# url-kaist/UV-SLAM

Hardware: AMD Instinct MI355X
Metric: sliding-window solves/sec (10 KF, 150 pts, 40 lines, 3 VP) (higher is better)
Workload: dtype f64; 1 GPU; W10-P150-L40-V3 x 256 independent windows per GPU (BASELINE configs[2]); single window (configs[1]) in single_window, the 20k-point window (configs[3]) in large_window (both with --full); windows_per_gpu=256, frames=11, points=150, lines=40, vp_tagged_lines=30, prior=True, parallelism=replicas x1

## Files before the change

### uv-slam_amd/csrc/uvs_solve_kernel.h

```cpp
#pragma once
#include <hip/hip_runtime.h>
#include "../../include/uvs_solver.h"
#include "uvs_layout.h"
#include "uvs_factors.h"

namespace uvsdev {


#ifndef UVS_X_PLAIN_TID
static __device__ __forceinline__ int lane_tid() { int t = threadIdx.x; asm volatile("" : "+v"(t)); return t; }
#else
static __device__ __forceinline__ int lane_tid() { return threadIdx.x; }
#endif
static constexpr int NT = UVS_NT;
static constexpr int NW = NT / 64;
static constexpr bool ROLES = NT > 256;
static constexpr int ET = ROLES ? 256 : NT;
static constexpr int EW = ET / 64;
static constexpr int GT0 = NT - UVS_GT;
UVS_DEV int wave_uniform() { return __builtin_amdgcn_readfirstlane((int)(threadIdx.x >> 6)); }
UVS_DEV bool role_eval() { return !ROLES || wave_uniform() < EW; }
#ifndef UVS_X_NO_LINE_ROTATE
UVS_DEV int line_lane() { return ROLES ? (lane_tid() ^ 256) : lane_tid(); }
#else
UVS_DEV int line_lane() { return lane_tid(); }
#endif
#define UVS_COST_LINE_LANE tid
#ifndef UVS_T_CP_PB
#define UVS_T_CP_PB 2
#define UVS_T_CP_LB 1
#define UVS_T_BS_LNB 4
#define UVS_T_PR_UN 26
#endif
static_assert(UVS_PT_C == UVS_PT_A + 12, "pt_anchor_pass reads A and c as one run");
static constexpr int CP_PB = NT > 256 ? UVS_T_CP_PB : 4;
static constexpr int CP_LB = NT > 256 ? UVS_T_CP_LB : 2;
static constexpr int BS_LNB = NT > 256 ? UVS_T_BS_LNB : 4;
static constexpr int PR_UN = NT > 256 ? UVS_T_PR_UN : 26;
static constexpr int PG_UN = NT > 256 ? 16 : 32;

static constexpr int L_X = 0;
static constexpr int L_XC = L_X + UVS_XDIM;
static constexpr int L_G = L_XC + UVS_XDIM;
static constexpr int L_DLT = L_G + UVS_RD;
static constexpr int L_HD = L_DLT + UVS_RD + 24;
static constexpr int L_SC = L_HD + UVS_RD;
static constexpr int L_DD = L_SC + UVS_RD;
static constexpr int L_DINV = L_DD + UVS_RD;
static constexpr int L_RF = L_DINV + UVS_RD;
static constexpr int L_EX = L_RF + 120;
static constexpr int L_PDX = L_EX + 16;
static constexpr int L_PR = L_PDX + UVS_MAX_PRIOR_DIM;
static constexpr int L_PRC = L_PR + UVS_MAX_PRIOR_DIM;
static constexpr int L_RED = L_PRC + UVS_MAX_PRIOR_DIM;
static constexpr int L_CTRL = L_RED + (5 * NW > 24 ? 5 * NW : 24);
static constexpr int L_PROF = L_CTRL + 32;
static constexpr int L_WPROF = L_PROF + 24;
static constexpr int L_LCOST = L_WPROF + 8;
static constexpr int LACC = 1;
static constexpr int L_LGMAX = L_LCOST + ET / LACC;
static constexpr int L_PX0 = L_LGMAX + 8;
static constexpr int L_PTAB = L_PX0 + 9 * UVS_MAX_PRIOR_BLOCKS;
static constexpr int L_SMALL = (L_PTAB + 2 * UVS_MAX_PRIOR_BLOCKS + 1) & ~1;
static constexpr int L_S = L_SMALL;
static constexpr int L_TOTAL = L_S + UVS_S_DOUBLES;
static_assert(L_TOTAL * 8 <= 160 * 1024, "LDS map exceeds the 160 KB of a CU");
enum { P_SETUP = 0, P_OBS, P_LMPREP, P_GATHER, P_ASSEMBLE, P_CHOL, P_TRSV, P_BACKSUB, P_COST, P_MISC, P_CH_DIAG, P_CH_PANEL, P_CH_TRAIL, P_AS_IMU, P_AS_ZERO, P_AS_ADD, P_LAST };
#define UVS_PROF(c, k) do { if ((c).o.debug && lane_tid() == 0) { const long long now_ = clock64(); (c).sh[L_PROF + (k)] += (double)(now_ - (long long)(c).sh[L_PROF + 23]); (c).sh[L_PROF + 23] = (double)now_; } } while (0)
static constexpr size_t LDS_BYTES = (size_t)L_TOTAL * 8;
static constexpr int TL_PER_WAVE = 4096;
__device__ long long g_lin_tl[8 * TL_PER_WAVE * 2];
#define UVS_TLOG(c, id) do { if ((c).o.debug == 5 && (threadIdx.x & 63) == 0 && blockIdx.x == 0) { const int w_ = threadIdx.x >> 6; const int n_ = (int)(c).sh[L_WPROF + w_]; \
    if (n_ < TL_PER_WAVE) { g_lin_tl[2 * (w_ * TL_PER_WAVE + n_)] = (id); g_lin_tl[2 * (w_ * TL_PER_WAVE + n_) + 1] = clock64(); (c).sh[L_WPROF + w_] = (double)(n_ + 1); } } } while (0)

enum { C_COST = 0, C_RADIUS, C_DECR, C_XNORM, C_GMAX, C_CAND, C_MCC, C_STEP2, C_XC2, C_GO, C_IT, C_INVALID, C_CUR, C_FIRST,
       C_TERM, C_NSUCC, C_CHOLOK, C_GMAXLM, C_TIMEUP };

struct KOpts {
    int max_it, ex_free, keep_cand, jacobi;
    double sqrt_info, line_factor, vp_factor, loss_pt, loss_ln, loss_vp, G[3];
    double r0, rmax, rmin, min_rel, dlo, dhi, ftol, gtol, ptol;
    int max_invalid;
    int debug;
    long long max_ticks;
    int redamp;
};

__constant__ unsigned char c_blk_fa[UVS_NBLK];
__constant__ unsigned char c_blk_fb[UVS_NBLK];

UVS_DEV int sidx(int i, int j) {
    const int bi = i >> 4, bj = j >> 4;
    return (((bi * (bi + 1)) >> 1) + bj) * UVS_BLK_SZ + (i & 15) * UVS_BLK_LD + (j & 15);
}
UVS_DEV double bcast_lane(double v, int lane) {
    const int lo = __builtin_amdgcn_readlane(__double2loint(v), lane);
    const int hi = __builtin_amdgcn_readlane(__double2hiint(v), lane);
    return __hiloint2double(hi, lo);
}
UVS_DEV void wave_sync() {
    __builtin_amdgcn_fence(__ATOMIC_RELEASE, "wavefront");
    __builtin_amdgcn_wave_barrier();
    __builtin_amdgcn_fence(__ATOMIC_ACQUIRE, "wavefront");
}

UVS_DEV double wave_sum(double v) {
#pragma unroll
    for (int off = 32; off > 0; off >>= 1) v += __shfl_down(v, off, 64);
    return v;
}
UVS_DEV double wave_max(double v) {
#pragma unroll
    for (int off = 32; off > 0; off >>= 1) v = fmax(v, __shfl_down(v, off, 64));
    return v;
}
UVS_DEV void rsqrt_pair(double x, double* sq, double* rsq) {
    const double y = __builtin_amdgcn_rsq(x);
    double g = x * y, hh = 0.5 * y;
    double r = fma(-hh, g, 0.5);
    g = fma(g, r, g); hh = fma(hh, r, hh);
    r = fma(-hh, g, 0.5);
    g = fma(g, r, g); hh = fma(hh, r, hh);
    const double d = fma(-g, g, x);
    g = fma(d, hh, g);
    *sq = g; *rsq = 2.0 * hh;
}
UVS_DEV void block_reduce(double* sh, double* s , double* mx) {
    const int tid = lane_tid(), lane = tid & 63, wv = tid >> 6;
    __syncthreads();
#pragma unroll
    for (int k = 0; k < 4; ++k) { const double t = wave_sum(s[k]); if (lane == 0) sh[L_RED + wv * 5 + k] = t; }
    { const double t = wave_max(*mx); if (lane == 0) sh[L_RED + wv * 5 + 4] = t; }
    __syncthreads();
    double a[4] = {0, 0, 0, 0}, m = 0.0;
#pragma unroll
    for (int w = 0; w < NW; ++w) {
#pragma unroll
        for (int k = 0; k < 4; ++k) a[k] += sh[L_RED + w * 5 + k];
        m = fmax(m, sh[L_RED + w * 5 + 4]);
    }
#pragma unroll
    for (int k = 0; k < 4; ++k) s[k] = a[k];
    *mx = m;
}

UVS_DEV void lacc_set(double* sh, double cost, double gmax) {
    const int tid = lane_tid();
    if (tid < ET) sh[L_LCOST + tid] = cost;
    const double wm = wave_max(gmax);
    if ((tid & 63) == 0) sh[L_LGMAX + (tid >> 6)] = wm;
}
UVS_DEV void lacc_add(double* sh, double cost, double gmax) {
    const int tid = lane_tid();
    if (tid < ET) sh[L_LCOST + tid] += cost;
    const double wm = wave_max(gmax);
    if ((tid & 63) == 0) sh[L_LGMAX + (tid >> 6)] = fmax(sh[L_LGMAX + (tid >> 6)], wm);
}
UVS_DEV double lacc_cost(const double* sh) { const int tid = lane_tid(); return tid < ET ? sh[L_LCOST + tid] : 0.0; }
UVS_DEV double lacc_gmax(const double* sh) { return sh[L_LGMAX + (lane_tid() >> 6)]; }

struct Ctx {
    const DevWin* hdr;
    const double* bd;
    const int* bi;
    double* ws;
    double* sh;
    KOpts o;
    int ltrig_ok = 0;
    int ptab_ok = 0;
};

UVS_DEV const double* line_trig_of(const Ctx& c, const double* line) {
    const DevWin& h = *c.hdr;
    if (!c.ltrig_ok) return nullptr;
    return line == c.ws + h.w_line0 ? c.ws + h.w_ltrig0 : (line == c.ws + h.w_line1 ? c.ws + h.w_ltrig1 : nullptr);
}

UVS_DEV void stage_rotations(const Ctx& c, const double* x) {
    const int tid = lane_tid();
    if (tid < UVS_NF) quat_to_R(x + 7 * tid + 3, c.sh + L_RF + 9 * tid);
    else if (tid == UVS_NF) { quat_to_R(x + 176 + 3, c.sh + L_EX); c.sh[L_EX + 9] = x[176]; c.sh[L_EX + 10] = x[177]; c.sh[L_EX + 11] = x[178]; }
    else if (tid == UVS_RELO_FRAME && c.hdr->relo_on) quat_to_R(x + 184 + 3, c.sh + L_RF + 9 * UVS_RELO_FRAME);
}
UVS_DEV const double* pose_of(const double* x, int f) { return x + (f > UVS_NF ? 184 : 7 * f); }

UVS_DEV void load_point_obs(const Ctx& c, int o, double td, double* pi, double* pj, double* vij) {
    const DevWin& h = *c.hdr;
    const double* m = c.bd + h.d_ptmeas + o; const int st = h.pt_stride;
    pi[0] = m[0]; pi[1] = m[st]; pi[2] = m[2 * st]; pj[0] = m[3 * st]; pj[1] = m[4 * st]; pj[2] = m[5 * st];
    if (h.td_on) {
        const double* v = c.bd + h.d_ptvel + o;
        vij[0] = v[0]; vij[1] = v[st]; vij[2] = v[2 * st]; vij[3] = v[3 * st];
        const double di = td - v[4 * st], dj = td - v[5 * st];
        pi[0] -= di * vij[0]; pi[1] -= di * vij[1]; pj[0] -= dj * vij[2]; pj[1] -= dj * vij[3];
    }
}

UVS_DEV void stage_prior_tables(const Ctx& c) {
    const int tid = lane_tid();
    const DevWin& h = *c.hdr;
    if (h.prior_n <= 0) return;
    int* tab = (int*)(c.sh + L_PTAB);
    if (tid < 4 * UVS_MAX_PRIOR_BLOCKS) tab[tid] = c.bi[h.i_prior + tid];
    if (tid < 9 * UVS_MAX_PRIOR_BLOCKS) c.sh[L_PX0 + tid] = c.bd[h.d_prior + h.prior_n * h.prior_n + 2 * h.prior_n + tid];
}
UVS_DEV void prior_dx(const Ctx& c, const double* x) {
    const int tid = lane_tid() - 64;
    const DevWin& h = *c.hdr;
    if (h.prior_n > 0 && tid >= 0 && tid < h.prior_nb) {
        int kind, frame, size, idx;
        double x0[9];
        if (c.ptab_ok) {
            const int* tab = (const int*)(c.sh + L_PTAB);
            kind = tab[tid]; frame = tab[16 + tid]; size = tab[32 + tid]; idx = tab[48 + tid];
#pragma unroll
            for (int k = 0; k < 9; ++k) x0[k] = c.sh[L_PX0 + 9 * tid + k];
        } else {
            const int* pt = c.bi + h.i_prior;
            kind = pt[tid]; frame = pt[16 + tid]; size = pt[32 + tid]; idx = pt[48 + tid];
            const double* x0g = c.bd + h.d_prior + h.prior_n * h.prior_n + 2 * h.prior_n + 9 * tid;
#pragma unroll
            for (int k = 0; k < 9; ++k) x0[k] = x0g[k];
        }
        const double* xb = (kind == UVS_BLOCK_POSE) ? x + 7 * frame : (kind == UVS_BLOCK_SPEEDBIAS) ? x + 77 + 9 * frame : (kind == UVS_BLOCK_TD) ? x + 183 : x + 176;
        double* dx = c.sh + L_PDX + idx;
        if (size != 7) { for (int k = 0; k < size; ++k) dx[k] = xb[k] - x0[k]; }
        else {
            dx[0] = xb[0] - x0[0]; dx[1] = xb[1] - x0[1]; dx[2] = xb[2] - x0[2];
            double qi[4], e[4]; quat_inv(x0 + 3, qi); quat_mul(qi, xb + 3, e);
            const double sg = (e[3] >= 0.0) ? 2.0 : -2.0;
            dx[3] = sg * e[0]; dx[4] = sg * e[1]; dx[5] = sg * e[2];
        }
    }
}
UVS_DEV double prior_quad(const Ctx& c, int dst = L_PR) {
    const DevWin& h = *c.hdr;
    const int n = h.prior_n, tid = lane_tid();
    double cost = 0.0;
    if (n <= 0) return cost;
    const double* H0 = c.ws + h.w_prior_h0;
    const int parts = (NT / n) < 4 ? (NT / n) : 4;
    const int part = tid / n, row = tid - part * n;
    const double g0v = tid < n ? c.ws[h.w_prior_h0 + UVS_PH_G0(n) + tid] : 0.0, c0v = tid == 0 ? c.ws[h.w_prior_h0 + UVS_PH_C0(n)] : 0.0;
    if (part < parts) {
        const int kb = (n * part) / parts, ke = (n * (part + 1)) / parts;
        double p8[8] = {0, 0, 0, 0, 0, 0, 0, 0};
        for (int k = kb; k < ke; k += PR_UN) {
            double jv[PR_UN];
#pragma unroll
            for (int u = 0; u < PR_UN; ++u) jv[u] = H0[(k + u < ke ? k + u : kb) * n + row];
#pragma unroll
            for (int u = 0; u < PR_UN; ++u) if (k + u < ke) p8[u & 7] += jv[u] * c.sh[L_PDX + k + u];
        }
        c.sh[L_S + 128 * part + row] = ((p8[0] + p8[1]) + (p8[2] + p8[3])) + ((p8[4] + p8[5]) + (p8[6] + p8[7]));
    }
    __syncthreads();
    if (tid < n) {
        double y = c.sh[L_S + tid];
        for (int p = 1; p < parts; ++p) y += c.sh[L_S + 128 * p + tid];
        c.sh[dst + tid] = y;
        cost = c.sh[L_PDX + tid] * (g0v + 0.5 * y);
        if (tid == 0) cost += c0v;
    }
    return cost;
}
UVS_DEV double prior_cost_share(const Ctx& c, int src) {
    const DevWin& h = *c.hdr;
    const int n = h.prior_n, tid = lane_tid();
    double cost = 0.0;
    if (tid < n) {
        cost = c.sh[L_PDX + tid] * (c.ws[h.w_prior_h0 + UVS_PH_G0(n) + tid] + 0.5 * c.sh[src + tid]);
        if (tid == 0) cost += c.ws[h.w_prior_h0 + UVS_PH_C0(n)];
    }
    return cost;
}
UVS_DEV double prior_residual_rows(const Ctx& c) {
    const DevWin& h = *c.hdr;
    const int n = h.prior_n, tid = lane_tid();
    double cost = 0.0;
    if (tid < n) {
        const double* Jr = c.bd + h.d_prior + (size_t)tid * n;
        double s = c.bd[h.d_prior + n * n + tid];
        for (int k = 0; k < n; ++k) s += Jr[k] * c.sh[L_PDX + k];
        c.sh[L_PR + tid] = s;
        cost = 0.5 * s * s;
    }
    return cost;
}

UVS_DEV void cost_imu_raw(const Ctx& c, const double* x, int lane0) {
    const DevWin& h = *c.hdr;
    const int b = lane_tid() - lane0;
    double* rs = c.sh + L_S + 1024;
    if (b >= 0 && b < h.n_imu) {
        const int fi = c.bi[h.i_imu + 2 * b], skip = c.bi[h.i_imu + 2 * b + 1];
        if (!skip) {
            const double* blk = c.bd + h.d_imu + (size_t)b * UVS_IMU_STRIDE;
            double r[15];
            imu_raw(blk, blk + UVS_IMU_JAC, c.o.G, x + 7 * fi, x + 77 + 9 * fi, x + 7 * (fi + 1), x + 77 + 9 * (fi + 1), r, nullptr);
#pragma unroll
            for (int i = 0; i < 15; ++i) rs[16 * b + i] = r[i];
        }
    }
}
// ... 213 lines not shown
    double a0[4], b0[4], a1[4], b1[4];
#define UVS_CH_LOAD(AV, BV) { _Pragma("unroll") for (int q = 0; q < 4; ++q) { AV[q] = Ai[4 * q]; BV[q] = Bj[4 * q]; } Bj += UVS_BLK_SZ; Ai += astep; }
#define UVS_CH_MFMA(AV, BV) { _Pragma("unroll") for (int q = 0; q < 4; ++q) acc = TR ? __builtin_amdgcn_mfma_f64_16x16x4f64(BV[q], AV[q], acc, 0, 0, 1) : __builtin_amdgcn_mfma_f64_16x16x4f64(AV[q], BV[q], acc, 0, 0, 1); }
    UVS_CH_LOAD(a0, b0)
    for (int j = j0;;) {
        if (j + 1 < j1) UVS_CH_LOAD(a1, b1)
        UVS_CH_MFMA(a0, b0)
        if (++j >= j1) break;
        if (j + 1 < j1) UVS_CH_LOAD(a0, b0)
        UVS_CH_MFMA(a1, b1)
        if (++j >= j1) break;
    }
#undef UVS_CH_LOAD
#undef UVS_CH_MFMA
}
template <bool RHS>
UVS_DEV void chol_panel_pair(double* sh, int i1, int i2, int k, int lane, const double* Bw, const d4_t& av) {
    d4_t acc = {0.0, 0.0, 0.0, 0.0};
#pragma unroll
    for (int q = 0; q < 4; ++q) acc = __builtin_amdgcn_mfma_f64_16x16x4f64(av[q], Bw[q], acc, 0, 0, 0);
    chol_store_pair<RHS>(sh, i1, i2, k, lane, acc);
}

UVS_DEV void chol_panel_item(double* sh, int i, int k, int lane, const double* Bw) {
    const int li = lane & 15, lk = lane >> 4;
    d4_t acc = {0.0, 0.0, 0.0, 0.0};
    double av[4];
    if (i != UVS_NF) {
        const double* Ai = sblk(sh, i, k) + li * UVS_BLK_LD + lk;
#pragma unroll
        for (int q = 0; q < 4; ++q) av[q] = Ai[4 * q];
    } else {
#pragma unroll
        for (int q = 0; q < 4; ++q) { const double yv = sh[L_DLT + 16 * k + 4 * q + lk]; av[q] = (li == 0) ? yv : 0.0; }
    }
#pragma unroll
    for (int q = 0; q < 4; ++q) acc = __builtin_amdgcn_mfma_f64_16x16x4f64(av[q], Bw[q], acc, 0, 0, 0);
    chol_store_item(sh, i, k, lane, acc);
}
UVS_DEV void chol_panel_from(double* sh, int i, int k, int lane, const double* Bw, const d4_t& av) {
    d4_t acc = {0.0, 0.0, 0.0, 0.0};
#pragma unroll
    for (int q = 0; q < 4; ++q) acc = __builtin_amdgcn_mfma_f64_16x16x4f64(av[q], Bw[q], acc, 0, 0, 0);
    chol_store_item(sh, i, k, lane, acc);
}
UVS_DEV void chol_panel_operand(double* sh, int k, int lane, double* Bw) {
    const int li = lane & 15, lk = lane >> 4;
    const double* Dk = sblk(sh, k, k);
#pragma unroll
    for (int q = 0; q < 4; ++q) {
        const int m = 4 * q + lk;
        const double up = Dk[m * UVS_BLK_LD + li], dg = sh[L_DINV + 16 * k + li];
        Bw[q] = (m < li) ? up : (m == li ? dg : 0.0);
    }
}

template <bool half>
UVS_DEV void chol_factor_impl(double* sh, int debug) {
    MiniCtx c; c.sh = sh; c.o.debug = debug;
    const int tid = lane_tid(), lane = tid & 63;
    const int wv = __builtin_amdgcn_readfirstlane(tid >> 6);
    const int li = lane & 15, lk = lane >> 4;
    int* flg = (int*)(sh + L_XC);
    if (tid < 80) flg[tid] = 0;
    if (tid == 0) sh[L_CTRL + C_CHOLOK] = 1.0;
    UVS_PROF(c, P_MISC);
#ifndef UVS_X_CHOL_ALL_WORKERS
    constexpr bool chain_alone = ROLES;
#else
    constexpr bool chain_alone = false;
#endif
    constexpr int nwork = chain_alone ? NW - 2 : NW - 1;
    const int wrk = chain_alone ? (wv < 4 ? wv - 1 : wv - 2) : wv - 1;
    const bool idle_wave = chain_alone && wv == 4;
    long long tend_ = 0;
    d4_t Lt = {0.0, 0.0, 0.0, 0.0};
#define UVS_FLAG_WAIT(idx, val) while (__hip_atomic_load(flg + (idx), __ATOMIC_ACQUIRE, __HIP_MEMORY_SCOPE_WORKGROUP) < (val)) __builtin_amdgcn_s_sleep(1);
#define UVS_FLAG_SET(idx) if (lane == 0) __hip_atomic_store(flg + (idx), 1, __ATOMIC_RELEASE, __HIP_MEMORY_SCOPE_WORKGROUP);
    __syncthreads();
    for (int k = 0; k < UVS_NF; ++k) {
        double* Dk = sblk(sh, k, k);
        if (idle_wave) { if (!half && k > 0) __syncthreads(); continue; }
        if (!half) { if (k > 0) __syncthreads(); }
        else if (wv == 0) { if (k >= 2) UVS_FLAG_WAIT(32 + k, 1) }
        else if (k > 0) {
            if (lane == 0) __hip_atomic_fetch_add(flg + 64, 1, __ATOMIC_RELEASE, __HIP_MEMORY_SCOPE_WORKGROUP);
            UVS_FLAG_WAIT(64, nwork * k)
            UVS_FLAG_WAIT(48 + k - 1, 1)
        }
        const long long tw0_ = debug ? clock64() : 0;
        long long tl_ = tw0_;
#define UVS_TL(slot) if (debug == 4 && lane == 0) { const long long t_ = clock64(); sh[L_WPROF + slot] += (double)(t_ - tl_); tl_ = t_; }
        if (debug == 4 && tid == 0 && k > 0) sh[L_WPROF + 7] += (double)(tw0_ - tend_);
        if (wv == 0) {
            d4_t dacc = chol_load_item(sh, k, k, lane);
            if (k > 0) {
#pragma unroll
                for (int q = 0; q < 4; ++q) dacc = __builtin_amdgcn_mfma_f64_16x16x4f64(Lt[q], Lt[q], dacc, 0, 0, 1);
            }
            d4_t T;
            UVS_TL(0)
#pragma unroll
            for (int q = 0; q < 4; ++q) T[q] = (lk + 4 * q == li) ? 1.0 : 0.0;
            double ap_prev = 0.0;
            double pivs[4] = {1.0, 1.0, 1.0, 1.0};
#pragma unroll
            for (int j = 0; j < 16; j += 2) {
                const int reg = j >> 2, s0 = j & 3, s1 = s0 + 1;
                const double a00 = bcast_lane(dacc[reg], 16 * s0 + j), a10 = bcast_lane(dacc[reg], 16 * s0 + j + 1), a11 = bcast_lane(dacc[reg], 16 * s1 + j + 1);
                if (j > 0) T = __builtin_amdgcn_mfma_f64_16x16x4f64(ap_prev, T[(j - 2) >> 2], T, 0, 0, 0);
                const auto lo = __builtin_amdgcn_permlane16_swap(__double2loint(dacc[reg]), __double2loint(dacc[reg]), false, false);
                const auto hi = __builtin_amdgcn_permlane16_swap(__double2hiint(dacc[reg]), __double2hiint(dacc[reg]), false, false);
                const double rj = __hiloint2double(hi[0], lo[0]), rj1 = __hiloint2double(hi[1], lo[1]);
                const double y0 = __builtin_amdgcn_rcp(a00);
                const double e0 = fma(-a00, y0, 1.0), l0 = a10 * y0, w0s = -rj * y0;
                const double p0 = fma(e0, e0, e0);
                const double l10 = fma(l0, p0, l0), w0 = fma(w0s, p0, w0s);
                const double d2 = fma(-l10, a10, a11);
                const double t = fma(-l10, rj, rj1);
                const double y1 = __builtin_amdgcn_rcp(d2);
                const double e1 = fma(-d2, y1, 1.0), u1s = -t * y1;
                const double p1 = fma(e1, e1, e1);
                double u1 = fma(u1s, p1, u1s);
                u1 = (li > j + 1) ? u1 : 0.0;
                const double u0 = fma(-u1, l10, w0);
                const double ap = (lk == s0) ? ((li > j) ? u0 : 0.0) : ((lk == s1) ? u1 : 0.0);
                if (lk == s0) pivs[reg] = a00;
                if (lk == s1) pivs[reg] = d2;
                dacc = __builtin_amdgcn_mfma_f64_16x16x4f64(ap, dacc[reg], dacc, 0, 0, 0);
                ap_prev = ap;
            }
            T = __builtin_amdgcn_mfma_f64_16x16x4f64(ap_prev, T[3], T, 0, 0, 0);
            if (k > 0) UVS_FLAG_WAIT(16 + k, 1)
            const d4_t av = chol_load_item_t(sh, k + 1, k, lane);
#pragma unroll
            for (int q = 0; q < 4; ++q) {
                const int j = lk + 4 * q;
                double ljj, inv; rsqrt_pair(pivs[q], &ljj, &inv);
                Dk[li * UVS_BLK_LD + j] = (li > j) ? dacc[q] * inv : (li == j ? ljj : T[q] * inv);
                if (li == j) { sh[L_DINV + 16 * k + j] = inv; if (!(pivs[q] > 0.0)) sh[L_CTRL + C_CHOLOK] = 0.0; }
            }
            if (lane == 0) __hip_atomic_store(flg + k, 1, __ATOMIC_RELEASE, __HIP_MEMORY_SCOPE_WORKGROUP);
            UVS_TL(1)
            UVS_TL(2)
            double Bw[4]; chol_panel_operand(sh, k, lane, Bw);
            {
                Lt = d4_t{0.0, 0.0, 0.0, 0.0};
#pragma unroll
                for (int q = 0; q < 4; ++q) Lt = __builtin_amdgcn_mfma_f64_16x16x4f64(Bw[q], av[q], Lt, 0, 0, 0);
                if (k + 1 < UVS_NF) {
                    double* Lb = sblk(sh, k + 1, k) + li * UVS_BLK_LD + lk;
#pragma unroll
                    for (int q = 0; q < 4; ++q) Lb[4 * q] = Lt[q];
                } else if (li == 0) {
#pragma unroll
                    for (int q = 0; q < 4; ++q) sh[L_DLT + 16 * k + lk + 4 * q] = Lt[q];
                }
                UVS_FLAG_SET(48 + k)
            }
            UVS_TL(3)
            tend_ = tl_;
            if (debug == 1 && lane == 0) sh[L_WPROF + 4] += (double)(clock64() - tw0_);
        } else if (half) {
            const int nPA = (UVS_NF - k - 1) / 2;
            const int nAi = nPA > 0 ? nPA : ((k + 2 <= UVS_NF) ? 1 : 0);
            const int nPL = (UVS_NF - k) / 2;
            constexpr int w_la0 = 1 % nwork, w_single = 0;
            const int t0 = (wrk + nwork - (2 % nwork)) % nwork;
            d4_t hold[2];
            static_assert((UVS_NF / 2 + nwork - 1) / nwork <= 2, "last-term items of a column per worker");
            if (k > 0) {
                if (wrk == w_la0 && k + 1 < UVS_NF) {
                    const int i1 = k + 1, i2 = (i1 + 1 < UVS_NF) ? i1 + 1 : i1;
                    d4_t acc = chol_load_pair<true>(sh, i1, i2, k + 1, lane);
                    chol_update_pair<false, true>(sh, i1, i2, k + 1, 0, k, lane, acc);
                    chol_store_pair<true>(sh, i1, i2, k + 1, lane, acc);
                    UVS_FLAG_SET(32 + k + 1)
                }
                if (wrk == w_single) {
                    if (k + 1 < UVS_NF) {
                        d4_t acc = chol_load_pair<false>(sh, k + 1, k + 1, k, lane);
                        chol_update_pair<false, false>(sh, k + 1, k + 1, k, k - 1, k, lane, acc);
                        chol_store_pair<false>(sh, k + 1, k + 1, k, lane, acc);
                    } else {
                        d4_t acc = chol_load_item(sh, k + 1, k, lane);
                        chol_update_item(sh, k + 1, k, k - 1, k, lane, acc);
                        chol_store_item(sh, k + 1, k, lane, acc);
                    }
                    UVS_FLAG_SET(16 + k)
                }
#pragma unroll
                for (int n = 0; n < 2; ++n) {
                    const int t = t0 + n * nwork;
                    const int i1 = k + 2 + 2 * t, i2 = (i1 + 1 < UVS_NF) ? i1 + 1 : i1;
                    if (t < nPA) {
                        if (t == 0) { hold[n] = chol_load_pair_t<true>(sh, i1, i2, k, lane); chol_update_pair<true, true>(sh, i1, i2, k, k - 1, k, lane, hold[n]); }
                        else { hold[n] = chol_load_pair_t<false>(sh, i1, i2, k, lane); chol_update_pair<true, false>(sh, i1, i2, k, k - 1, k, lane, hold[n]); }
                    } else if (t < nAi) {
                        hold[n] = chol_load_item_t(sh, UVS_NF, k, lane);
                        chol_update_item<true>(sh, UVS_NF, k, k - 1, k, lane, hold[n]);
                    }
                }
                if (k + 1 < UVS_NF) {
                    int load[nwork];
#pragma unroll
                    for (int w = 0; w < nwork; ++w) {
                        const int tw = (w + nwork - (2 % nwork)) % nwork;
                        load[w] = (tw < nAi ? (nAi - tw + nwork - 1) / nwork : 0) * 17 + (w == w_la0 ? 5 + 4 * k : 0) + (w == w_single ? 9 : 0);
                    }
                    for (int u = 1; u < nPL; ++u) {
                        int best = 0;
#pragma unroll
                        for (int w = 1; w < nwork; ++w) if (load[w] < load[best]) best = w;
#pragma unroll
                        for (int w = 0; w < nwork; ++w) if (w == best) load[w] += 5 + 4 * k;
                        if (best == wrk) {
                            const int i1 = k + 1 + 2 * u, i2 = (i1 + 1 < UVS_NF) ? i1 + 1 : i1;
                            d4_t acc = chol_load_pair<false>(sh, i1, i2, k + 1, lane);
                            chol_update_pair<false, false>(sh, i1, i2, k + 1, 0, k, lane, acc);
                            chol_store_pair<false>(sh, i1, i2, k + 1, lane, acc);
                        }
                    }
                }
            }
            if (debug == 1 && lane == 0) sh[L_WPROF + 4 + wv] += (double)(clock64() - tw0_);
            if (wv == 1) UVS_TL(4)
            while (__hip_atomic_load(flg + k, __ATOMIC_ACQUIRE, __HIP_MEMORY_SCOPE_WORKGROUP) == 0) __builtin_amdgcn_s_sleep(1);
            if (wv == 1) UVS_TL(5)
            double Bw[4]; chol_panel_operand(sh, k, lane, Bw);
            if (k > 0) {
#pragma unroll
                for (int n = 0; n < 2; ++n) {
                    const int t = t0 + n * nwork;
                    const int i1 = k + 2 + 2 * t, i2 = (i1 + 1 < UVS_NF) ? i1 + 1 : i1;
                    if (t < nPA) { if (t == 0) chol_panel_pair<true>(sh, i1, i2, k, lane, Bw, hold[n]); else chol_panel_pair<false>(sh, i1, i2, k, lane, Bw, hold[n]); }
                    else if (t < nAi) chol_panel_from(sh, UVS_NF, k, lane, Bw, hold[n]);
                }
            } else {
                for (int t = t0; t < nPA; t += nwork) {
                    const int i1 = 2 + 2 * t, i2 = (i1 + 1 < UVS_NF) ? i1 + 1 : i1;
                    if (t == 0) { const d4_t av = chol_load_pair_t<true>(sh, i1, i2, 0, lane); chol_panel_pair<true>(sh, i1, i2, 0, lane, Bw, av); }
                    else { const d4_t av = chol_load_pair_t<false>(sh, i1, i2, 0, lane); chol_panel_pair<false>(sh, i1, i2, 0, lane, Bw, av); }
                }
            }
            if (wv == 1) UVS_TL(6)
        } else {
            d4_t hold[3];
            static_assert((UVS_NF - 2 + nwork - 1) / nwork <= 3, "rows of a column (k > 0) per worker");
            if (k > 0) {
                int light = 0, best = 1 << 30;
#pragma unroll
                for (int w = 0; w < nwork; ++w) {
                    const int na = UVS_NF - k - 1 - w, nl = (k + 1 < UVS_NF) ? UVS_NF - k - (nwork - 1 - w) : 0;
                    const int ca = na > 0 ? (na + nwork - 1) / nwork : 0, cl = nl > 0 ? (nl + nwork - 1) / nwork : 0;
                    const int load = ca * 17 + cl * (5 + 4 * k);
                    if (load < best) { best = load; light = w; }
                }
                if (wrk == light) {
                    d4_t acc = chol_load_item(sh, k + 1, k, lane);
                    chol_update_item(sh, k + 1, k, k - 1, k, lane, acc);
                    chol_store_item(sh, k + 1, k, lane, acc);
                    if (lane == 0) __hip_atomic_store(flg + 16 + k, 1, __ATOMIC_RELEASE, __HIP_MEMORY_SCOPE_WORKGROUP);
                }
#pragma unroll
                for (int n = 0; n < 3; ++n) {
                    const int i = k + 2 + wrk + n * nwork;
                    if (i <= UVS_NF) { hold[n] = chol_load_item_t(sh, i, k, lane); chol_update_item<true>(sh, i, k, k - 1, k, lane, hold[n]); }
                }
                if (k + 1 < UVS_NF) {
                    for (int i = k + 1 + (nwork - 1 - wrk); i <= UVS_NF; i += nwork) {
                        d4_t acc = chol_load_item(sh, i, k + 1, lane);
                        chol_update_item(sh, i, k + 1, 0, k, lane, acc);
                        chol_store_item(sh, i, k + 1, lane, acc);
                    }
                }
            }
            if (debug == 1 && lane == 0) sh[L_WPROF + 4 + wv] += (double)(clock64() - tw0_);
            if (wv == 1) UVS_TL(4)
            while (__hip_atomic_load(flg + k, __ATOMIC_ACQUIRE, __HIP_MEMORY_SCOPE_WORKGROUP) == 0) __builtin_amdgcn_s_sleep(1);
            if (wv == 1) UVS_TL(5)
            double Bw[4]; chol_panel_operand(sh, k, lane, Bw);
            if (k > 0) {
#pragma unroll
                for (int n = 0; n < 3; ++n) { const int i = k + 2 + wrk + n * nwork; if (i <= UVS_NF) chol_panel_from(sh, i, k, lane, Bw, hold[n]); }
            } else {
                for (int i = 2 + wrk; i <= UVS_NF; i += nwork) chol_panel_item(sh, i, k, lane, Bw);
            }
            if (wv == 1) UVS_TL(6)
        }
        UVS_PROF(c, P_CH_DIAG);
    }
    __syncthreads();
}
__device__ __attribute__((noinline)) void chol_factor_call(int debug) {
    extern __shared__ __attribute__((aligned(16))) double sh_chol[];
    chol_factor_impl<true>(sh_chol, debug);
}
__device__ __attribute__((noinline)) void chol_factor_call_full_rows(int debug) {
    extern __shared__ __attribute__((aligned(16))) double sh_chol[];
    chol_factor_impl<false>(sh_chol, debug);
}
UVS_DEV void chol_factor(const Ctx& c) { if (c.hdr->chol_half_ok) chol_factor_call(c.o.debug); else chol_factor_call_full_rows(c.o.debug); }

UVS_DEV void chol_solve_impl(double* sh) {
    const int tid = lane_tid();
    double* b = sh + L_DLT;
    __syncthreads();
    if (tid < 64) {
        for (int k = UVS_NF - 1; k >= 0; --k) {
            const double* Dk = sblk(sh, k, k);
            const int c16 = tid & 15;
            double wv_[16], rv[16];
#pragma unroll
            for (int m = 0; m < 16; ++m) { wv_[m] = Dk[c16 * UVS_BLK_LD + m]; rv[m] = b[16 * k + m]; }
            const double dinv = sh[L_DINV + 16 * k + c16];
            double p4[4] = {0.0, 0.0, 0.0, 0.0};
#pragma unroll
            for (int m = 0; m < 16; ++m) { const double w = (m > c16) ? wv_[m] : (m == c16 ? dinv : 0.0); p4[m & 3] += w * rv[m]; }
            const double s = (p4[0] + p4[1]) + (p4[2] + p4[3]);
            wave_sync();
            if (tid < 16) b[16 * k + tid] = s;
            wave_sync();
            double xk[16];
#pragma unroll
            for (int r = 0; r < 16; ++r) xk[r] = b[16 * k + r];
            for (int t = tid; t < 16 * k; t += 64) {
                const int j = t >> 4, cc = t & 15;
                const double* B = sblk(sh, k, j) + cc;
                double bv[16];
#pragma unroll
                for (int r = 0; r < 16; ++r) bv[r] = B[r * UVS_BLK_LD];
                double u4[4] = {0.0, 0.0, 0.0, 0.0};
#pragma unroll
                for (int r = 0; r < 16; ++r) u4[r & 3] += bv[r] * xk[r];
                b[16 * j + cc] -= (u4[0] + u4[1]) + (u4[2] + u4[3]);
            }
            wave_sync();
        }
    }
    __syncthreads();
}
UVS_DEV void chol_solve(const Ctx& c) { chol_solve_impl(c.sh); }

static constexpr int GRP_PER_WAVE = 64 / UVS_GLANES;
static constexpr int GR = UVS_GROWS;
static constexpr int LIST_HDR = 2 * (UVS_NGRP + 1);
typedef double d2_t __attribute__((ext_vector_type(2)));

struct GAcc { double v[6 * GR], g[GR], hd[GR]; };

UVS_DEV d2_t lds2(const double* p) { return *(const d2_t*)p; }
UVS_DEV void gacc_gather_parts(GAcc& A, int grp, double* scr) {
    const int tid = lane_tid() - GT0;
    const int part = grp >= 0 ? (grp >> 9) & 15 : 0, np = grp >= 0 ? ((grp >> 21) & 15) + 1 : 1;
    constexpr int NV = 8 * GR, LD = NV + 1;
    double* D = scr + LD * tid;
    if (np > 1) {
#pragma unroll
        for (int q = 0; q < 6 * GR; ++q) D[q] = A.v[q];
#pragma unroll
        for (int q = 0; q < GR; ++q) { D[6 * GR + q] = A.g[q]; D[7 * GR + q] = A.hd[q]; }
    }
    __syncthreads();
    if (np > 1) {
        const double* D0 = D - LD * UVS_GLANES * part;
        for (int q = part; q < NV; q += np) {
            double sacc = D0[q];
            for (int p = 1; p < np; ++p) sacc += D0[LD * UVS_GLANES * p + q];
            const_cast<double*>(D0)[q] = sacc;
        }
    }
    __syncthreads();
    if (np > 1 && part == 0) {
#pragma unroll
        for (int q = 0; q < 6 * GR; ++q) A.v[q] = D[q];
#pragma unroll
        for (int q = 0; q < GR; ++q) { A.g[q] = D[6 * GR + q]; A.hd[q] = D[7 * GR + q]; }
    }
}
UVS_DEV void gacc_zero(GAcc& A) {
#pragma unroll
    for (int q = 0; q < 6 * GR; ++q) A.v[q] = 0.0;
#pragma unroll
    for (int q = 0; q < GR; ++q) { A.g[q] = 0.0; A.hd[q] = 0.0; }
}
UVS_DEV void row_fma(double* v, double s, const d2_t* q) {
    v[0] += s * q[0].x; v[1] += s * q[0].y; v[2] += s * q[1].x; v[3] += s * q[1].y; v[4] += s * q[2].x; v[5] += s * q[2].y;
}

UVS_DEV int gather_group(const Ctx& c) { const int t = lane_tid() - GT0; return t >= 0 ? c.bi[c.hdr->i_wblk + (t / UVS_GLANES)] : -1; }

template <int K, class Ops, class Load, class Use>
UVS_DEV void gather_walk(const int* ent, int e0, int e1, Load load, Use use) {
    if (e0 >= e1) return;
    Ops A, B;
    int wa[K], wb[K];
    const auto fetch = [&](int i, int* w) {
#pragma unroll
        for (int u = 0; u < K; ++u) w[u] = ent[i + u < e1 ? i + u : e0];
    };
    fetch(e0, wa); load(e0, wa, A); fetch(e0 + K, wb);
    for (int i = e0;;) {
        load(i + K, wb, B); fetch(i + 2 * K, wa);
        use(i, A);
        i += K; if (i >= e1) break;
        load(i + K, wa, A); fetch(i + 2 * K, wb);
        use(i, B);
        i += K; if (i >= e1) break;
    }
}

template <bool EXT, bool DELTA = false>
UVS_DEV void gather_points(int grp, const int* lists, const double* S0, GAcc& A, int goff = 0, bool exrows = true) {
    const int g = (lane_tid() - GT0) / UVS_GLANES, r0 = GR * (lane_tid() % UVS_GLANES);
    const bool on = grp >= 0;
    const bool diag = on && ((grp >> 8) & 1);
    const bool tdg = EXT && on && ((grp >> 13) & 15) == UVS_NF;
    const bool exg = EXT && exrows && on && ((grp >> 13) & 15) == UVS_NF + 1;
    const bool tdcol = exg && ((grp >> 17) & 15) == UVS_NF;
    const int p1off = tdg ? 1 : 6, rcoff = tdg ? UVS_PT_RC2 - UVS_PT_TD : exg ? UVS_PT_RC2 - UVS_PT_EX : 12;
    const bool dirv = !(tdg && diag) && !tdcol;
    const int* ent = lists + LIST_HDR;
    {
        struct Ops { double ea[2][GR]; d2_t q[2][3]; double gg[2][DELTA ? GR : 1]; };
        const int e0 = on ? lists[g] : 0, e1 = on ? lists[g + 1] : 0;
        gather_walk<2, Ops>(ent, e0, e1,
            [&](int, const int* w, Ops& o) {
#pragma unroll
                for (int u = 0; u < 2; ++u) {
                    const double* pa = S0 + (w[u] & 0x7fff) + r0;
                    const double* pb = S0 + ((unsigned)w[u] >> 16);
#pragma unroll
                    for (int r = 0; r < GR; ++r) o.ea[u][r] = pa[r];
                    o.q[u][0] = lds2(pb); o.q[u][1] = lds2(pb + 2); o.q[u][2] = lds2(pb + 4);
                    if (DELTA) {
#pragma unroll
                        for (int r = 0; r < GR; ++r) o.gg[u][r] = pa[goff + r];
                    }
                }
            },
            [&](int i, Ops& o) {
#pragma unroll
                for (int u = 0; u < 2; ++u) {
                    const bool ok = i + u < e1;
#pragma unroll
                    for (int r = 0; r < GR; ++r) row_fma(A.v + 6 * r, ok ? -o.ea[u][r] : 0.0, o.q[u]);
                    if (DELTA) {
#pragma unroll
                        for (int r = 0; r < GR; ++r) A.g[r] -= (ok && diag) ? o.gg[u][r] : 0.0;
                    }
                }
            });
    }
    if (DELTA) return;
    {
        struct Ops { double p0[GR], p1[GR]; d2_t q0[3], q1[3], rc; };
        const int e0 = on ? lists[UVS_NGRP + 1 + g] : 0, e1 = on ? lists[UVS_NGRP + 2 + g] : 0;
        gather_walk<1, Ops>(ent, e0, e1,
            [&](int, const int* w, Ops& o) {
                const int lo = w[0] & 0x7fff;
                const double* pa = S0 + lo + r0;
                const double* pb = S0 + ((unsigned)w[0] >> 16);
#pragma unroll
                for (int r = 0; r < GR; ++r) { o.p0[r] = pa[r]; o.p1[r] = pa[p1off + r]; }
#pragma unroll
                for (int k = 0; k < 3; ++k) { o.q0[k] = lds2(pb + 2 * k); o.q1[k] = lds2(pb + 6 + 2 * k); }
                o.rc = lds2(S0 + lo + ((w[0] & UVS_PT_ENTRY_A) ? UVS_PT_RC2 - UVS_PT_A : rcoff));
            },
            [&](int, Ops& o) {
#pragma unroll
                for (int r = 0; r < GR; ++r) {
                    if (dirv) { row_fma(A.v + 6 * r, o.p0[r], o.q0); row_fma(A.v + 6 * r, o.p1[r], o.q1); }
                    if (tdcol) A.v[6 * r] += o.p0[r] * o.q0[0].x + o.p1[r] * o.q0[0].y;
                    if (diag) { A.g[r] += o.p0[r] * o.rc.x + o.p1[r] * o.rc.y; A.hd[r] += o.p0[r] * o.p0[r] + o.p1[r] * o.p1[r]; }
                }
            });
    }
}

template <bool DELTA = false>
UVS_DEV void gather_lines(int grp, const int* lists, const double* S0, GAcc& A, int goff = 0, int eoff = 0) {
    const int g = (lane_tid() - GT0) / UVS_GLANES, r0 = GR * (lane_tid() % UVS_GLANES);
    const bool on = grp >= 0;
    const bool diag = on && ((grp >> 8) & 1);
    const int* ent = lists + LIST_HDR;
    {
        struct Ops { double ea[4][GR]; d2_t y[4][3]; double gg[DELTA ? GR : 1]; };
        const int e0 = on ? lists[g] : 0, e1 = on ? lists[g + 1] : 0;
        gather_walk<1, Ops>(ent, e0, e1,
            [&](int, const int* w, Ops& o) {
                const int lo = w[0] & 0x7fff;
                const double* pa = S0 + lo + r0;
                const double* pb = S0 + ((unsigned)w[0] >> 16);
#pragma unroll
                for (int q = 0; q < 4; ++q) {
#pragma unroll
                    for (int r = 0; r < GR; ++r) o.ea[q][r] = pa[6 * q + r];
                    o.y[q][0] = lds2(pb + 6 * q); o.y[q][1] = lds2(pb + 6 * q + 2); o.y[q][2] = lds2(pb + 6 * q + 4);
                }
                if (DELTA) {
                    const double* pg = S0 + goff + 6 * ((lo - eoff) / UVS_LN_EY) + r0;
#pragma unroll
                    for (int r = 0; r < GR; ++r) o.gg[r] = pg[r];
                }
            },
            [&](int, Ops& o) {
#pragma unroll
                for (int q = 0; q < 4; ++q)
#pragma unroll
                    for (int r = 0; r < GR; ++r) row_fma(A.v + 6 * r, -o.ea[q][r], o.y[q]);
                if (DELTA) {
#pragma unroll
                    for (int r = 0; r < GR; ++r) A.g[r] -= diag ? o.gg[r] : 0.0;
                }
            });
    }
    if (DELTA) return;
    {
        struct Ops { double p[3][GR]; d2_t q[3][3], rc01; double rc2; };
        const int e0 = on ? lists[UVS_NGRP + 1 + g] : 0, e1 = on ? lists[UVS_NGRP + 2 + g] : 0;
        gather_walk<1, Ops>(ent, e0, e1,
            [&](int, const int* w, Ops& o) {
                const double* R = S0 + w[0];
#pragma unroll
                for (int k = 0; k < 3; ++k) {
#pragma unroll
                    for (int r = 0; r < GR; ++r) o.p[k][r] = R[UVS_LN_JP + 6 * k + r0 + r];
                    o.q[k][0] = lds2(R + UVS_LN_JP + 6 * k); o.q[k][1] = lds2(R + UVS_LN_JP + 6 * k + 2); o.q[k][2] = lds2(R + UVS_LN_JP + 6 * k + 4);
                }
                o.rc01 = lds2(R); o.rc2 = R[UVS_LN_RV];
            },
            [&](int, Ops& o) {
#pragma unroll
                for (int r = 0; r < GR; ++r) {
#pragma unroll
                    for (int k = 0; k < 3; ++k) { row_fma(A.v + 6 * r, o.p[k][r], o.q[k]); A.hd[r] += o.p[k][r] * o.p[k][r]; }
                    A.g[r] += o.p[0][r] * o.rc01.x + o.p[1][r] * o.rc01.y + o.p[2][r] * o.rc2;
                }
            });
    }
}

static constexpr int IMU_JLD = 48;
static constexpr int IMU_WOFF = 16 * IMU_JLD;
static constexpr int IMU_BLK = IMU_WOFF + UVS_BLK_SZ;
#ifndef UVS_IMU_SLOT_SWAP
#define UVS_IMU_SLOT_SWAP 1
#endif
static constexpr int IMU_SLOTS = (UVS_NF - 1 + NW - 1) / NW;
UVS_DEV int imu_block_of(int wv, int s) {
    if (NW == 8 && UVS_IMU_SLOT_SWAP) return s == 0 ? wv : (wv == 0 ? 9 : wv == 1 ? 8 : UVS_NF);
    return wv + s * NW;
}
struct ImuN { d4_t n00[IMU_SLOTS], n10[IMU_SLOTS], n11[IMU_SLOTS]; int fi[IMU_SLOTS]; bool act[IMU_SLOTS]; };

UVS_DEV double lin_prep(const Ctx& c, const double* x, int mode = 0) {
    UVS_PROF(c, P_MISC);
    const int tid = lane_tid(), n = c.hdr->prior_n;
    if (mode == 0) {
        stage_rotations(c, x);
        prior_dx(c, x);
        __syncthreads();
        return prior_quad(c);
    }
    if (mode == 2) { stage_rotations(c, x); prior_dx(c, x); __syncthreads(); }
    else if (tid < n) c.sh[L_PR + tid] = c.sh[L_PRC + tid];
    __syncthreads();
    return prior_cost_share(c, L_PR);
}
UVS_DEV void lin_imu_stage(const Ctx& c, const double* x) {
    const DevWin& h = *c.hdr;
    double* sh = c.sh;
    const int tid = lane_tid(), lane = tid & 63, wv = tid >> 6;
    __syncthreads();
    UVS_PROF(c, P_GATHER);
    double* IM = sh + L_S;
    constexpr int WPL = ((UVS_NF - 1) * 225 + ET - 1) / ET;
    double wreg[WPL];
#pragma unroll
    for (int q = 0; q < WPL; ++q) {
        const int t = tid + q * ET, tc = t < h.n_imu * 225 ? t : 0, b = tc / 225, e = tc - 225 * b;
        wreg[q] = c.ws[h.w_imu_w + (size_t)b * UVS_IMU_WS + e];
    }
    for (int t = tid; t < h.n_imu * IMU_BLK; t += ET) IM[t] = 0.0;
    UVS_TLOG(c, 40);
    __syncthreads();
    UVS_TLOG(c, 41);
    if (lane < h.n_imu && wv < 4 && !c.bi[h.i_imu + 2 * lane + 1]) {
        const int fi = c.bi[h.i_imu + 2 * lane];
        const double* blk = c.bd + h.d_imu + (size_t)lane * UVS_IMU_STRIDE;
        double* T = IM + IMU_BLK * lane;
        const double* pi_ = x + 7 * fi; const double* si_ = x + 77 + 9 * fi; const double* pj_ = x + 7 * (fi + 1); const double* sj_ = x + 77 + 9 * (fi + 1);
        double r[15];
        if (EW < 4) { imu_raw<IMU_JLD, 1, false>(blk, blk + UVS_IMU_JAC, c.o.G, pi_, si_, pj_, sj_, r, T); for (int i = 0; i < 15; ++i) T[i * IMU_JLD + 31] = r[i]; }
        else if (wv == 0) { imu_raw<IMU_JLD, 1, false, 1>(blk, blk + UVS_IMU_JAC, c.o.G, pi_, si_, pj_, sj_, r, T); for (int i = 0; i < 15; ++i) T[i * IMU_JLD + 31] = r[i]; }
        else if (wv == 1) imu_raw<IMU_JLD, 1, false, 2>(blk, blk + UVS_IMU_JAC, c.o.G, pi_, si_, pj_, sj_, r, T);
        else if (wv == 2) imu_raw<IMU_JLD, 1, false, 4>(blk, blk + UVS_IMU_JAC, c.o.G, pi_, si_, pj_, sj_, r, T);
        else imu_raw<IMU_JLD, 1, false, 8>(blk, blk + UVS_IMU_JAC, c.o.G, pi_, si_, pj_, sj_, r, T);
    }
#pragma unroll
    for (int q = 0; q < WPL; ++q) {
        const int t = tid + q * ET;
        if (t < h.n_imu * 225) { const int b = t / 225, e = t - 225 * b, i = e / 15, k = e - 15 * i; IM[IMU_BLK * b + IMU_WOFF + i * UVS_BLK_LD + k] = wreg[q]; }
    }
    UVS_TLOG(c, 42);
    __syncthreads();
    UVS_TLOG(c, 43);
}
UVS_DEV double lin_imu_tiles(const Ctx& c, ImuN& N) {
    const DevWin& h = *c.hdr;
    double* sh = c.sh;
    const int tid = lane_tid(), lane = tid & 63, wv = tid >> 6, li = lane & 15, lk = lane >> 4;
    double cost = 0.0;
    double* IM = sh + L_S;
    bool act[IMU_SLOTS];
#pragma unroll
    for (int s = 0; s < IMU_SLOTS; ++s) {
        const int b = imu_block_of(wv, s);
        act[s] = b < h.n_imu && !c.bi[h.i_imu + 2 * (b < h.n_imu ? b : 0) + 1];
        N.act[s] = act[s]; N.fi[s] = c.bi[h.i_imu + 2 * (b < h.n_imu ? b : 0)];
        if (act[s]) {
            double* Jb = IM + IMU_BLK * b; const double* Wb = Jb + IMU_WOFF;
            d4_t t0 = {0.0, 0.0, 0.0, 0.0}, t1 = t0;
            double wa[4], j0[4], j1[4];
#pragma unroll
            for (int q = 0; q < 4; ++q) { wa[q] = Wb[li * UVS_BLK_LD + 4 * q + lk]; j0[q] = Jb[(4 * q + lk) * IMU_JLD + li]; j1[q] = Jb[(4 * q + lk) * IMU_JLD + 16 + li]; }
#pragma unroll
            for (int q = 0; q < 4; ++q) { t0 = __builtin_amdgcn_mfma_f64_16x16x4f64(wa[q], j0[q], t0, 0, 0, 0); t1 = __builtin_amdgcn_mfma_f64_16x16x4f64(wa[q], j1[q], t1, 0, 0, 0); }
#pragma unroll
            for (int q = 0; q < 4; ++q) { Jb[(lk + 4 * q) * IMU_JLD + li] = t0[q]; Jb[(lk + 4 * q) * IMU_JLD + 16 + li] = t1[q]; }
        }
    }
    wave_sync();
#pragma unroll
    for (int s = 0; s < IMU_SLOTS; ++s) {
        const int b = imu_block_of(wv, s);
        d4_t n00 = {0.0, 0.0, 0.0, 0.0}, n10 = n00, n11 = n00;
        if (act[s]) {
            const double* Jb = IM + IMU_BLK * b;
            double j0[4], j1[4];
#pragma unroll
            for (int q = 0; q < 4; ++q) { j0[q] = Jb[(4 * q + lk) * IMU_JLD + li]; j1[q] = Jb[(4 * q + lk) * IMU_JLD + 16 + li]; }
#pragma unroll
            for (int q = 0; q < 4; ++q) {
                n00 = __builtin_amdgcn_mfma_f64_16x16x4f64(j0[q], j0[q], n00, 0, 0, 0);
// ... 1624 lines not shown
```

Baseline: 179,400 solves/s.

## Keep Cholesky back-substitution vector in registers using cross-lane permutes

Replaces the LDS-based block back-substitution with a register-resident solve. Each of the 64 lanes holds up to three slots of the right-hand side, and row values are broadcast across lanes with permlane16/32 swaps and DPP. The recursion is compile-time unrolled over frames, prefetches the next blocks and skips zero half-rows when the factor is half-populated. This removes the per-step LDS round trips and wave syncs in the serial triangular solve, at the cost of heavy template unrolling, inline DPP asm and higher register pressure. The old path stays available behind a macro.

Result: faster. 182,800 solves/s (median of 6 runs) (+1.9%).

```diff
diff --git a/uv-slam_amd/csrc/uvs_solve_kernel.h b/uv-slam_amd/csrc/uvs_solve_kernel.h
--- a/uv-slam_amd/csrc/uvs_solve_kernel.h
+++ b/uv-slam_amd/csrc/uvs_solve_kernel.h
@@ -1,5 +1,6 @@
 #pragma once
 #include <hip/hip_runtime.h>
+#include <utility>
 #include "../../include/uvs_solver.h"
 #include "uvs_layout.h"
 #include "uvs_factors.h"
@@ -819,6 +820,7 @@
 }
 UVS_DEV void chol_factor(const Ctx& c) { if (c.hdr->chol_half_ok) chol_factor_call(c.o.debug); else chol_factor_call_full_rows(c.o.debug); }
 
+#ifdef UVS_X_TRSV_LDS
 UVS_DEV void chol_solve_impl(double* sh) {
     const int tid = lane_tid();
     double* b = sh + L_DLT;
@@ -858,6 +860,125 @@
     __syncthreads();
 }
 UVS_DEV void chol_solve(const Ctx& c) { chol_solve_impl(c.sh); }
+#else
+template <int Q> UVS_DEV double trsv_row_all(double v) {
+    const unsigned lo = (unsigned)__double2loint(v), hi = (unsigned)__double2hiint(v);
+    const auto hl = __builtin_amdgcn_permlane32_swap(lo, lo, false, false);
+    const auto hh = __builtin_amdgcn_permlane32_swap(hi, hi, false, false);
+    const auto al = __builtin_amdgcn_permlane16_swap(hl[Q >> 1], hl[Q >> 1], false, false);
+    const auto ah = __builtin_amdgcn_permlane16_swap(hh[Q >> 1], hh[Q >> 1], false, false);
+    return __hiloint2double((int)ah[Q & 1], (int)al[Q & 1]);
+}
+UVS_DEV double trsv_rows_sum(double v) {
+    const unsigned lo = (unsigned)__double2loint(v), hi = (unsigned)__double2hiint(v);
+    const auto al = __builtin_amdgcn_permlane16_swap(lo, lo, false, false);
+    const auto ah = __builtin_amdgcn_permlane16_swap(hi, hi, false, false);
+    const double t = __hiloint2double((int)ah[0], (int)al[0]) + __hiloint2double((int)ah[1], (int)al[1]);
+    const unsigned tlo = (unsigned)__double2loint(t), thi = (unsigned)__double2hiint(t);
+    const auto bl = __builtin_amdgcn_permlane32_swap(tlo, tlo, false, false);
+    const auto bh = __builtin_amdgcn_permlane32_swap(thi, thi, false, false);
+    return __hiloint2double((int)bh[0], (int)bl[0]) + __hiloint2double((int)bh[1], (int)bl[1]);
+}
+template <int M> UVS_DEV double trsv_row_lane(double v) {
+    return __builtin_amdgcn_update_dpp(0.0, v, 0x150 + M, 0xf, 0xf, true);
+}
+UVS_DEV double trsv_quad_rotate(double v) {
+    int lo = __double2loint(v), hi = __double2hiint(v);
+    const int l0 = lo, h0 = hi;
+    lo = __builtin_amdgcn_update_dpp(lo, l0, 0x55, 0x2, 0xf, false); hi = __builtin_amdgcn_update_dpp(hi, h0, 0x55, 0x2, 0xf, false);
+    lo = __builtin_amdgcn_update_dpp(lo, l0, 0xaa, 0x4, 0xf, false); hi = __builtin_amdgcn_update_dpp(hi, h0, 0xaa, 0x4, 0xf, false);
+    lo = __builtin_amdgcn_update_dpp(lo, l0, 0xff, 0x8, 0xf, false); hi = __builtin_amdgcn_update_dpp(hi, h0, 0xff, 0x8, 0xf, false);
+    return __hiloint2double(hi, lo);
+}
+template <int R> UVS_DEV double trsv_fmac_row_lane(double acc, double a, double x) {
+    asm("v_fmac_f64_dpp %0, %2, %1 row_newbcast:%3 row_mask:0xf bank_mask:0xf" : "+v"(acc) : "v"(a), "v"(x), "n"(R));
+    return acc;
+}
+UVS_DEV double trsv_dpp_source(double x) { asm volatile("s_nop 1" : "+v"(x)); return x; }
+template <bool HALF, int K, int T> struct TrsvTrip {
+    static constexpr int QL = (K - 1) & 3;
+    static constexpr bool last = (T == ((K - 1) >> 2));
+    static constexpr bool far_only = (4 * T + 3 < K - 1);
+    static constexpr bool live(int r) { return !(HALF && far_only && r >= 6 && r < 15); }
+    template <int R> static UVS_DEV void term(double* u4, const double* bv, double x) { if constexpr (live(R)) u4[R & 3] = trsv_fmac_row_lane<R>(u4[R & 3], bv[R], x); }
+    template <int... R> static UVS_DEV void terms(double* u4, const double* bv, double x, std::integer_sequence<int, R...>) { (term<R>(u4, bv, x), ...); }
+    static UVS_DEV void load(double* sh, int c16, int q, double* bv) {
+        const int qc = (last && q > QL) ? QL : q;
+        const double* B = sblk(sh, K, 4 * T) + qc * UVS_BLK_SZ + c16;
+#pragma unroll
+        for (int r = 0; r < 16; ++r) if (live(r)) bv[r] = B[r * UVS_BLK_LD];
+    }
+    static UVS_DEV void apply(int q, const double* bv, double x, double& bslot) {
+        double u4[4] = {0.0, 0.0, 0.0, 0.0};
+        terms(u4, bv, x, std::make_integer_sequence<int, 16>());
+        const double nb = bslot - ((u4[0] + u4[1]) + (u4[2] + u4[3]));
+        bslot = (!last || q <= QL) ? nb : bslot;
+    }
+};
+template <int K> UVS_DEV void trsv_load_w(double* sh, int c16, int q, double* w) {
+    const double* Dk = sblk(sh, K, K) + c16 * UVS_BLK_LD + q;
+#pragma unroll
+    for (int i = 0; i < 4; ++i) w[i] = Dk[4 * i];
+    w[4] = sh[L_DINV + 16 * K + c16];
+}
+template <bool HALF, int K>
+UVS_DEV void trsv_steps(double* sh, int c16, int q, double* bs, const int* msk, int eq, const double* wK) {
+    constexpr int SK = K >> 2, QK = K & 3, S1 = (K - 1) >> 2;
+    double bv0[16], bv1[16], bv2[16], wN[5];
+    if constexpr (K > 0) {
+        TrsvTrip<HALF, K, S1>::load(sh, c16, q, bv0);
+        if constexpr (S1 > 0) TrsvTrip<HALF, K, S1 - 1>::load(sh, c16, q, bv1);
+        if constexpr (S1 > 1) TrsvTrip<HALF, K, S1 - 2>::load(sh, c16, q, bv2);
+        trsv_load_w<K - 1>(sh, c16, q, wN);
+    }
+    double rv[4];
+    const double cur = trsv_row_all<QK>(bs[SK]);
+    const double rot = trsv_quad_rotate(cur);
+    rv[0] = trsv_row_lane<0>(rot); rv[1] = trsv_row_lane<4>(rot); rv[2] = trsv_row_lane<8>(rot); rv[3] = trsv_row_lane<12>(rot);
+    double p = fma(__builtin_amdgcn_ldexp(wK[4], eq), cur, 0.0);
+#pragma unroll
+    for (int i = 0; i < 4; ++i) p += __builtin_amdgcn_ldexp(wK[i], msk[i]) * rv[i];
+    const double s = trsv_dpp_source(trsv_rows_sum(p));
+    bs[SK] = (q == QK) ? s : bs[SK];
+    if constexpr (K > 0) {
+        TrsvTrip<HALF, K, S1>::apply(q, bv0, s, bs[S1]);
+        if constexpr (S1 > 0) TrsvTrip<HALF, K, S1 - 1>::apply(q, bv1, s, bs[S1 - 1]);
+        if constexpr (S1 > 1) TrsvTrip<HALF, K, S1 - 2>::apply(q, bv2, s, bs[S1 - 2]);
+        static_assert(S1 <= 2, "at most three update trips per step");
+        trsv_steps<HALF, K - 1>(sh, c16, q, bs, msk, eq, wN);
+    }
+}
+template <bool HALF>
+UVS_DEV void chol_solve_impl(double* sh) {
+    const int tid = lane_tid();
+    double* b = sh + L_DLT;
+    static_assert(UVS_NF >= 2 && UVS_NF <= 12 && UVS_RD > 128 && UVS_RD <= 192, "three register slots of 64 unknowns");
+    __syncthreads();
+    if (tid < 64) {
+        const int c16 = tid & 15, q = tid >> 4;
+        double bs[3] = {b[tid], b[64 + tid], (128 + tid < UVS_RD) ? b[128 + tid] : 0.0};
+        int msk[4];
+#pragma unroll
+        for (int i = 0; i < 4; ++i) msk[i] = (4 * i + q > c16) ? 0 : -4096;
+        const int eq = ((c16 & 3) == q) ? 0 : -4096;
+        double w0[5];
+        trsv_load_w<UVS_NF - 1>(sh, c16, q, w0);
+        trsv_steps<HALF, UVS_NF - 1>(sh, c16, q, bs, msk, eq, w0);
+        b[tid] = bs[0]; b[64 + tid] = bs[1];
+        if (128 + tid < UVS_RD) b[128 + tid] = bs[2];
+    }
+    __syncthreads();
+}
+__device__ __attribute__((noinline)) void chol_solve_call() {
+    extern __shared__ __attribute__((aligned(16))) double sh_chol[];
+    chol_solve_impl<true>(sh_chol);
+}
+__device__ __attribute__((noinline)) void chol_solve_call_full_rows() {
+    extern __shared__ __attribute__((aligned(16))) double sh_chol[];
+    chol_solve_impl<false>(sh_chol);
+}
+UVS_DEV void chol_solve(const Ctx& c) { if (c.hdr->chol_half_ok) chol_solve_call(); else chol_solve_call_full_rows(); }
+#endif
 
 static constexpr int GRP_PER_WAVE = 64 / UVS_GLANES;
 static constexpr int GR = UVS_GROWS;
```
